# ibrahimhroob/SPS

Hardware: AMD Instinct MI355X
Metric: scans/sec @100k pts, 0.1 m voxel (higher is better)
Workload: dtype f32; 1 GPU; BASELINE config 2: single ~100k-pt LiDAR-like scan + variant-B submap, 0.1 m voxel, CustomMinkUNet14 fp32, 1 scan per step per GPU (4 distinct scans cycled); scan_points=100824, rows=153557, streams_per_gpu=8, compact_arenas=True

## Files before the change

sps_amd/csrc/conv_kernels.inc.h:

```cpp

typedef float floatx4 __attribute__((ext_vector_type(4)));

struct ConvArgs {
  const float *in;
  float *out;
  const float *Wu;
  const float *scale;
  const float *shift;
  const float *res;
  const int *nbr;
  const uint32_t *tmask;
  const int *n_out;
  const int *abort_flag;
  int out_rows;
  int64_t ldn;
  int ldi, ldo, ldr;
  int K, cin, cout, NT, upk;
  int relu, S;
  float inv_upk;
  float in_const;
  uint32_t in_bytes, wu_bytes, nbr_bytes;
  int tile_cap;
  int trace_on;
  const float *in2;
// ... 706 lines not shown
        yv[i] = y;
        if (UP) acc_s[0][rr * AST + col] = y;
      }
      if (ro < count && c0 < a.cout) {
        float *__restrict__ op = a.out + (size_t)ro * a.ldo + c0;
        if constexpr (EP_CPT == 2) *reinterpret_cast<float2 *>(op) = make_float2(yv[0], yv[1]);
        else *reinterpret_cast<float4 *>(op) = make_float4(yv[0], yv[1], yv[2], yv[3]);
      }
      if (FIN) {
#pragma unroll
        for (int o = 1; o < EP_TPR; o <<= 1) fsum += __shfl_xor(fsum, o, 64);
        if ((threadIdx.x % EP_TPR) == 0 && ro < count) a.fin_out[ro] = fsum + a.fin_b;
      }
    }
    if constexpr (UP) {
      __syncthreads();
      const __amdgpu_buffer_rsrc_t rsU = __builtin_amdgcn_make_buffer_rsrc((void *)a.up_Wu, 0, (int)a.up_wu_bytes, 0x00020000);
      const float usc = n < a.up_cout ? a.up_scale[n] : 0.f, ush = n < a.up_cout ? a.up_shift[n] : 0.f;
      const __amdgpu_buffer_rsrc_t rsUm = __builtin_amdgcn_make_buffer_rsrc((void *)a.up_tmask, 0, (int)0xFFFFFFFEu, 0x00020000);
      uint32_t om[4];
      const uint32_t omv = __builtin_amdgcn_raw_buffer_load_b32(rsUm, row0 + 16 * q < count ? (uint32_t)(st * 4 + q) * 16u : 0xFFFFFFFFu, 0, 0) & 0xFFu;
#pragma unroll
      for (int t = 0; t < 4; ++t) om[t] = (uint32_t)__builtin_amdgcn_readlane((int)omv, 16 * t);
#pragma unroll
      for (int kk = 0; kk < 2; ++kk) {
        const int k = 2 * wave + kk;
        if (!(((om[0] | om[1] | om[2] | om[3]) >> k) & 1u)) continue;
        const u32x4 vb = __builtin_amdgcn_raw_buffer_load_b128(rsU, (uint32_t)(k * 4 + q) * 256u + (uint32_t)n * 16u, 0, 0);
#pragma unroll
        for (int t = 0; t < 4; ++t) {
          if (!((om[t] >> k) & 1u)) continue;
          int child[4];
          {
            const int4 cv4 = *reinterpret_cast<const int4 *>(a.up_down + (size_t)k * a.up_ldn + row0 + 16 * t + q * 4);
            const int cv[4] = {cv4.x, cv4.y, cv4.z, cv4.w};
#pragma unroll
            for (int i = 0; i < 4; ++i) {
              const int ro = row0 + 16 * t + q * 4 + i;
              child[i] = ro < count ? cv[i] : -1;
              if (child[i] >= a.up_rows) child[i] = -1;
            }
          }
          const floatx4 xa = *reinterpret_cast<const floatx4 *>(acc_s[0] + (16 * t + n) * AST + 4 * q);
          floatx4 d = floatx4{0.f, 0.f, 0.f, 0.f};
          d = __builtin_amdgcn_mfma_f32_16x16x4f32(xa.x, __uint_as_float(vb.x), d, 0, 0, 0);
          d = __builtin_amdgcn_mfma_f32_16x16x4f32(xa.y, __uint_as_float(vb.y), d, 0, 0, 0);
          d = __builtin_amdgcn_mfma_f32_16x16x4f32(xa.z, __uint_as_float(vb.z), d, 0, 0, 0);
          d = __builtin_amdgcn_mfma_f32_16x16x4f32(xa.w, __uint_as_float(vb.w), d, 0, 0, 0);
          if (n < a.up_cout) {
#pragma unroll
            for (int i = 0; i < 4; ++i)
              if (child[i] >= 0) a.up_out[(size_t)child[i] * a.up_ldo + n] = fmaxf(d[i] * usc + ush, 0.f);
          }
        }
      }
    }
    PX_STAMP(6);
#if defined(SPS_WAVE_TRACE)
    if (tr_on && lane == 0 && st < 4096) {
      tr[7] = ((unsigned long long)nch << 32) | (unsigned)st;
      if (wave < 4) for (int i = 0; i < 8; ++i) g_px_trace[(st * 4 + wave) * 8 + i] = tr[i];
    }
#endif
    __syncthreads();
  }
}

template <int NT>
__global__ __launch_bounds__(256) void k_upconv(ConvArgs a) {
  if (a.abort_flag && *a.abort_flag) return;
  const int count = *a.n_out;
  const int ntiles = (count + 15) >> 4;
  const int lane = threadIdx.x & 63, wave = __builtin_amdgcn_readfirstlane((int)(threadIdx.x >> 6));
  const int r = lane & 15, q = lane >> 4;
  const __amdgpu_buffer_rsrc_t rsA = __builtin_amdgcn_make_buffer_rsrc((void *)a.in, 0, (int)a.in_bytes, 0x00020000);
  const __amdgpu_buffer_rsrc_t rsW = __builtin_amdgcn_make_buffer_rsrc((void *)a.Wu, 0, (int)a.wu_bytes, 0x00020000);
  const int upk = a.upk;
  const int ngrp = (upk + 3) >> 2;
  float esc[NT], esh[NT];
#pragma unroll
  for (int nt = 0; nt < NT; ++nt) {
    const int col = nt * 16 + r;
    esc[nt] = col < a.cout ? a.scale[col] : 0.f;
    esh[nt] = col < a.cout ? a.shift[col] : 0.f;
  }
  for (int tile = blockIdx.x; tile < ntiles; tile += gridDim.x) {
    const int row0 = tile * 16;
    const uint32_t mask = a.tmask[(size_t)tile * 4] & 0xFFu;
    const int row = row0 + r;
    u32x4 va[4];
#pragma unroll
    for (int i = 0; i < 4; ++i) {
      const uint32_t oa = (i < ngrp && 4 * i + q < upk && row < count) ? (uint32_t)row * ((uint32_t)a.ldi * 4u) + (uint32_t)(4 * i + q) * 16u : OOR;
      va[i] = __builtin_amdgcn_raw_buffer_load_b128(rsA, oa, 0, 0);
    }
#pragma unroll
    for (int kk = 0; kk < 2; ++kk) {
      const int k = 2 * wave + kk;
      if (!((mask >> k) & 1u)) continue;
      int child[4];
      {
        const int4 cv4 = *reinterpret_cast<const int4 *>(a.nbr + (size_t)k * a.ldn + row0 + q * 4);
        const int cv[4] = {cv4.x, cv4.y, cv4.z, cv4.w};
#pragma unroll
        for (int i = 0; i < 4; ++i) {
          const int ro = row0 + q * 4 + i;
          child[i] = ro < count ? cv[i] : -1;
          if (a.out_rows > 0 && child[i] >= a.out_rows) child[i] = -1;
        }
      }
      floatx4 acc[NT];
#pragma unroll
      for (int nt = 0; nt < NT; ++nt) acc[nt] = floatx4{0.f, 0.f, 0.f, 0.f};
#pragma unroll
      for (int i = 0; i < 4; ++i) {
        if (i >= ngrp) break;
        const uint32_t ob = 4 * i + q < upk ? ((uint32_t)(k * upk + 4 * i + q) * (uint32_t)NT) * 256u + (uint32_t)r * 16u : OOR;
        u32x4 vb[NT];
#pragma unroll
        for (int nt = 0; nt < NT; ++nt) vb[nt] = __builtin_amdgcn_raw_buffer_load_b128(rsW, ob + nt * 256u, 0, 0);
#pragma unroll
        for (int nt = 0; nt < NT; ++nt) {
          acc[nt] = __builtin_amdgcn_mfma_f32_16x16x4f32(__uint_as_float(va[i].x), __uint_as_float(vb[nt].x), acc[nt], 0, 0, 0);
          acc[nt] = __builtin_amdgcn_mfma_f32_16x16x4f32(__uint_as_float(va[i].y), __uint_as_float(vb[nt].y), acc[nt], 0, 0, 0);
          acc[nt] = __builtin_amdgcn_mfma_f32_16x16x4f32(__uint_as_float(va[i].z), __uint_as_float(vb[nt].z), acc[nt], 0, 0, 0);
          acc[nt] = __builtin_amdgcn_mfma_f32_16x16x4f32(__uint_as_float(va[i].w), __uint_as_float(vb[nt].w), acc[nt], 0, 0, 0);
        }
      }
      const __amdgpu_buffer_rsrc_t rsR = __builtin_amdgcn_make_buffer_rsrc((void *)(a.res ? a.res : a.out), 0, (int)0xFFFFFFFEu, 0x00020000);
#pragma unroll
      for (int nt = 0; nt < NT; ++nt) {
        const int col = nt * 16 + r;
        if (col >= a.cout) continue;
        float rv[4] = {0.f, 0.f, 0.f, 0.f};
        if (a.res) {
#pragma unroll
          for (int i = 0; i < 4; ++i)
            rv[i] = __uint_as_float(__builtin_amdgcn_raw_buffer_load_b32(
                rsR, child[i] >= 0 ? ((uint32_t)child[i] * (uint32_t)a.ldr + (uint32_t)col) * 4u : 0xFFFFFFFFu, 0, 0));
        }
#pragma unroll
        for (int i = 0; i < 4; ++i) {
          if (child[i] < 0) continue;
          float y = acc[nt][i] * esc[nt] + esh[nt];
          y += rv[i];
          if (a.relu) y = fmaxf(y, 0.f);
          a.out[(size_t)child[i] * a.ldo + col] = y;
        }
      }
    }
  }
}

__global__ __launch_bounds__(256) void k_conv0_fused(const int *__restrict__ n_out, LevelView L,
                                                      const float *__restrict__ W, const float *__restrict__ scale,
                                                      const float *__restrict__ shift, float in_const,
                                                      float *__restrict__ out, int ldo, int relu, TileOrderArgs to, int g0) {
  __shared__ float w_s[128 * 8];
  const int gto = (int)gridDim.x - g0;
  if ((int)blockIdx.x < gto) {
    const int which = (int)blockIdx.x;
    if (which < NLV - TILE_ORDER_FIRST_LEVEL)
      tile_order_body(to, which);
    else
      px_order_body(to, which - (NLV - TILE_ORDER_FIRST_LEVEL));
    return;
  }
  const int bid = (int)blockIdx.x - gto;
  if (n_out[ABORT]) return;
  for (int i = threadIdx.x; i < 128 * 8; i += blockDim.x) w_s[i] = i < 125 * 8 ? W[i] : 0.f;
  __syncthreads();
  const int n = *n_out;
  const int ntiles = (n + 15) >> 4;
  const int lane = threadIdx.x & 63, wave = __builtin_amdgcn_readfirstlane((int)(threadIdx.x >> 6));
  const int r = lane & 15, q = lane >> 4;
  const float esc = r < 8 ? scale[r] : 0.f, esh = r < 8 ? shift[r] : 0.f;
  const __amdgpu_buffer_rsrc_t rsM = __builtin_amdgcn_make_buffer_rsrc((void *)L.bmask, 0, (int)0xFFFFFFFEu, 0x00020000);
  for (int tile = bid * 4 + wave; tile < ntiles; tile += g0 * 4) {
    const int row0 = tile * 16;
    const int u = row0 + r;
    uint32_t bm[4] = {0u, 0u, 0u, 0u};
#if defined(SPS_ABLATE_C0FETCH)
    bm[0] = bm[1] = 0x0F0F0F0Fu;
    if (false) {
      const int blk = L.vblock[u];
#else
    if (u < n) {
      const int blk = L.vblock[u];
#endif
      const int bit = L.vbit[u];
      const int px = bit & 3, py = (bit >> 2) & 3, pz = bit >> 4;
      const int lx = px < 2 ? -1 : 0, ly = py < 2 ? -1 : 0, lz = pz < 2 ? -1 : 0;
      const int ysel = q & 1, zsel = q >> 1;
      const int *adj = L.badj + (size_t)blk * 81 + 27 + (lz + zsel + 1) * 9 + (ly + ysel + 1) * 3 + (lx + 1);
      const int nb0 = adj[0], nb1 = adj[1];
      const u32x2 M0 = __builtin_amdgcn_raw_buffer_load_b64(rsM, nb0 >= 0 ? (uint32_t)nb0 * 8u : 0xFFFFFFFFu, 0, 0);
      const u32x2 M1 = __builtin_amdgcn_raw_buffer_load_b64(rsM, nb1 >= 0 ? (uint32_t)nb1 * 8u : 0xFFFFFFFFu, 0, 0);
      const uint32_t m0lo = M0.x, m0hi = M0.y, m1lo = M1.x, m1hi = M1.y;
      const int ysplit = 4 * (ly + 1), zsplit = 4 * (lz + 1);
      const int ty0 = ysel ? ysplit : py - 2, ty1 = ysel ? py + 2 : ysplit - 1;
      const int tz0 = zsel ? zsplit : pz - 2, tz1 = zsel ? pz + 2 : zsplit - 1;
      const int xs = px - 2 - 4 * lx;
#pragma unroll 1
      for (int iz = 0; iz < 4; ++iz) {
        const int tz = tz0 + iz;
        const bool hiw = (tz & 2) != 0;
        const uint32_t w0 = hiw ? m0hi : m0lo, w1 = hiw ? m1hi : m1lo;
        uint32_t plane = 0u;
#pragma unroll
        for (int iy = 0; iy < 4; ++iy) {
          const int ty = ty0 + iy;
          const bool on = tz <= tz1 && ty <= ty1;
          const int sh = ((tz & 1) << 4) | ((ty & 3) << 2);
          const uint32_t n0 = (w0 >> sh) & 0xFu, n1 = (w1 >> sh) & 0xFu;
          const uint32_t pres = on ? (((n0 | (n1 << 4)) >> xs) & 0x1Fu) : 0u;
          plane |= pres << (5 * iy);
        }
        const int k0 = 5 * ((ty0 - py + 2) + 5 * (tz - pz + 2));
        const unsigned long long wide = (unsigned long long)plane << (k0 & 31);
        const int wi = (k0 >> 5) & 3;
        bm[0] |= wi == 0 ? (uint32_t)wide : 0u;
        bm[1] |= wi == 1 ? (uint32_t)wide : (wi == 0 ? (uint32_t)(wide >> 32) : 0u);
        bm[2] |= wi == 2 ? (uint32_t)wide : (wi == 1 ? (uint32_t)(wide >> 32) : 0u);
        bm[3] |= wi == 3 ? (uint32_t)wide : (wi == 2 ? (uint32_t)(wide >> 32) : 0u);
      }
    }
#pragma unroll
    for (int w = 0; w < 4; ++w) {
      bm[w] |= __shfl_xor(bm[w], 16, 64);
      bm[w] |= __shfl_xor(bm[w], 32, 64);
    }
    floatx4 acc = floatx4{0.f, 0.f, 0.f, 0.f};
    uint32_t bq[4];
#pragma unroll
    for (int w = 0; w < 4; ++w) bq[w] = bm[w] >> q;
    const uint32_t cbits = __float_as_uint(in_const);
#pragma unroll
    for (int g = 0; g < 32; ++g) {
      const int k = 4 * g + q;
      const float av = __uint_as_float((uint32_t)__builtin_amdgcn_sbfe((int)bq[g >> 3], (4 * g) & 31, 1) & cbits);
      const float bv = r < 8 ? w_s[k * 8 + r] : 0.f;
      acc = __builtin_amdgcn_mfma_f32_16x16x4f32(av, bv, acc, 0, 0, 0);
    }
    if (r < 8) {
#pragma unroll
      for (int i = 0; i < 4; ++i) {
        const int ro = row0 + q * 4 + i;
        if (ro < n) {
          const float y = acc[i] * esc + esh;
          out[(size_t)ro * ldo + r] = relu ? fmaxf(y, 0.f) : y;
        }
      }
    }
  }
}


constexpr double FEAT_FIX = 4294967296.0;

__global__ void k_voxel_feat_accum(const float *__restrict__ feats, const int *__restrict__ inv, int n,
                                   long long *__restrict__ vacc, int *__restrict__ vcnt, const int *__restrict__ n_dev) {
  if (n_dev) n = min(n, *n_dev);
  const int p = blockIdx.x * blockDim.x + threadIdx.x;
  if (p >= n) return;
  const int v = inv[p];
  if (v < 0) return;
  const double f = fmin(fmax((double)feats[p], -32768.0), 32768.0);
  atomicAdd(reinterpret_cast<unsigned long long *>(vacc) + v, (unsigned long long)__double2ll_rn(f * FEAT_FIX));
  atomicAdd(vcnt + v, 1);
}

__global__ void k_voxel_feat_mean(const int *__restrict__ n_vox, const long long *__restrict__ vacc,
                                  const int *__restrict__ vcnt, float *__restrict__ vfeat) {
  if (n_vox[ABORT]) return;
  const int n = *n_vox;
  for (int v = blockIdx.x * blockDim.x + threadIdx.x; v < n; v += gridDim.x * blockDim.x)
    vfeat[v] = (float)(((double)vacc[v] / FEAT_FIX) / (double)max(vcnt[v], 1));
}

__global__ __launch_bounds__(256) void k_conv0_feat(const int *__restrict__ n_out, LevelView L,
                                                     const float *__restrict__ W, const float *__restrict__ scale,
                                                     const float *__restrict__ shift,
                                                     const float *__restrict__ vfeat, float *__restrict__ out,
                                                     int ldo, TileOrderArgs to, int g0) {
  __shared__ float w_s[128 * 8];
  __shared__ float val_s[4][16][132];
  const int gto = (int)gridDim.x - g0;
  if ((int)blockIdx.x < gto) {
    const int which = (int)blockIdx.x;
    if (which < NLV - TILE_ORDER_FIRST_LEVEL)
      tile_order_body(to, which);
    else
      px_order_body(to, which - (NLV - TILE_ORDER_FIRST_LEVEL));
    return;
  }
  const int bid = (int)blockIdx.x - gto;
  if (n_out[ABORT]) return;
  for (int i = threadIdx.x; i < 128 * 8; i += blockDim.x) w_s[i] = i < 125 * 8 ? W[i] : 0.f;
  __syncthreads();
  const int n = *n_out;
  const int ntiles = (n + 15) >> 4;
  const int lane = threadIdx.x & 63, wave = __builtin_amdgcn_readfirstlane((int)(threadIdx.x >> 6));
  const int r = lane & 15, q = lane >> 4;
  const float esc = r < 8 ? scale[r] : 0.f, esh = r < 8 ? shift[r] : 0.f;
  float *va = val_s[wave][r];
  for (int tile = bid * 4 + wave; tile < ntiles; tile += g0 * 4) {
    const int row0 = tile * 16;
    const int u = row0 + r;
    __builtin_amdgcn_wave_barrier();
    for (int j = q; j < 128; j += 4) va[j] = 0.f;
    __builtin_amdgcn_wave_barrier();
    if (u < n) {
      const int blk = L.vblock[u];
      const int bit = L.vbit[u];
      const int px = bit & 3, py = (bit >> 2) & 3, pz = bit >> 4;
      const int *adj = L.badj + (size_t)blk * 81;
      for (int c = q; c < 25; c += 4) {
        const int ty = py + c % 5 - 2, tz = pz + c / 5 - 2;
        const int ad0 = 27 + ((tz >> 2) + 1) * 9 + ((ty >> 2) + 1) * 3 + 1;
        const int nbit0 = ((tz & 3) << 4) | ((ty & 3) << 2);
        int last_bo = 99, base = 0;
        unsigned long long mk = 0ull;
#pragma unroll
        for (int dx = -2; dx <= 2; ++dx) {
          const int tx = px + dx;
          const int bo = tx >> 2;
          if (bo != last_bo) {
            last_bo = bo;
            const int nb = adj[ad0 + bo];
            mk = nb >= 0 ? L.bmask[nb] : 0ull;
            base = nb >= 0 ? L.bbase[nb] : 0;
          }
          const int nbit = nbit0 | (tx & 3);
          if ((mk >> nbit) & 1ull) va[5 * c + dx + 2] = vfeat[base + __popcll(mk & ((1ull << nbit) - 1ull))];
        }
      }
    }
    __builtin_amdgcn_wave_barrier();
    floatx4 acc = floatx4{0.f, 0.f, 0.f, 0.f};
#pragma unroll
    for (int g = 0; g < 32; ++g) {
      const int k = 4 * g + q;
      const float av = va[k];
      const float bv = r < 8 ? w_s[k * 8 + r] : 0.f;
      acc = __builtin_amdgcn_mfma_f32_16x16x4f32(av, bv, acc, 0, 0, 0);
    }
    if (r < 8) {
#pragma unroll
      for (int i = 0; i < 4; ++i) {
        const int ro = row0 + q * 4 + i;
        if (ro < n) out[(size_t)ro * ldo + r] = fmaxf(acc[i] * esc + esh, 0.f);
      }
    }
  }
}

__global__ void k_slice_head(const float *__restrict__ F, int ldf, const int *__restrict__ inv, int n,
                             const float *__restrict__ W, const float *__restrict__ bias, int oc, int act,
                             float *__restrict__ out, int64_t ldo, const int *__restrict__ abort_flag,
                             const int *__restrict__ n_dev) {
  if (n_dev) n = min(n, *n_dev);
  const int p = blockIdx.x * blockDim.x + threadIdx.x;
  if (p >= n) return;
  const int v = (abort_flag && *abort_flag) ? -1 : inv[p];
  float f[8];
  if (v >= 0) {
    const float4 a = *reinterpret_cast<const float4 *>(F + (size_t)v * ldf);
    const float4 b = *reinterpret_cast<const float4 *>(F + (size_t)v * ldf + 4);
    f[0] = a.x, f[1] = a.y, f[2] = a.z, f[3] = a.w, f[4] = b.x, f[5] = b.y, f[6] = b.z, f[7] = b.w;
  }
  for (int j = 0; j < oc; ++j) {
    float y = __builtin_nanf("");
    if (v >= 0) {
      y = 0.f;
#pragma unroll
      for (int c = 0; c < 8; ++c) y += f[c] * W[c * oc + j];
      y += bias[j];
      if (act == 1) y = 1.0f / (1.0f + expf(-y));
    }
    out[(size_t)p * ldo + j] = y;
  }
}

__global__ void k_slice_sigmoid(const float *__restrict__ logits, const int *__restrict__ inv, int n,
                                float *__restrict__ scores, const int *__restrict__ abort_flag) {
  const int p = blockIdx.x * blockDim.x + threadIdx.x;
  if (p >= n) return;
  const int v = (abort_flag && *abort_flag) ? -1 : inv[p];
  scores[p] = v >= 0 ? 1.0f / (1.0f + expf(-logits[v])) : __builtin_nanf("");
}

__global__ __launch_bounds__(256) void k_bhash_cleanup(PyramidArgs pa, int gb) {
  bhash_cleanup(pa, (int)blockIdx.x / gb, (int)blockIdx.x % gb, gb);
}
```

sps_amd/csrc/sps_hip.hip:

```cpp
#include <hip/hip_runtime.h>

#include <cmath>
#include <cstdarg>
#include <cstdint>
#include <cstdio>
#include <algorithm>
#include <array>
#include <cstdlib>
#include <cstring>
#include <map>
#include <memory>
#include <string>
#include <vector>

#include "../../include/sps_hip.h"

#if !defined(SPS_DIAG)
#undef SPS_ABLATE_A
#undef SPS_ABLATE_B
#undef SPS_ABLATE_HALF_B
#undef SPS_ABLATE_SKIP_B
#undef SPS_ABLATE_MFMA
#undef SPS_ABLATE_LOOP
#undef SPS_ABLATE_STAGE
// ... 430 lines not shown

PyramidArgs pyramid_args(sps_ctx *c) {
  PyramidArgs a{};
  for (int l = 0; l < NLV; ++l) {
    const Level &L = c->lv[l];
    a.h[l] = L.h;
    a.sslot[l] = L.sslot;
    a.bslot[l] = L.bslot;
    a.bkey[l] = L.bkey;
    a.bmask[l] = L.bmask;
    a.bbase[l] = L.bbase;
    a.bmb[l] = L.bmb;
    a.bparent[l] = L.bparent;
    a.bchild[l] = L.bchild;
    a.badj[l] = L.badj;
    a.vblock[l] = L.vblock;
    a.vbit[l] = L.vbit;
  }
  a.counts = c->counts;
  a.sbit0 = c->lv[0].sbit;
  a.agg = c->scan_agg;
  a.agg_stride = (int)(c->cap / SCAN_BLOCK + 8);
  a.gen = (uint32_t)(c->fwd_gen % 0xFFFFFFFFull) + 1u;
  a.n_dev = nullptr;
  for (int l = 0; l < NLV; ++l) {
    a.capl[l] = (int)c->capl[l];
    a.bcapl[l] = (int)c->bcapl[l];
  }
  a.err = c->err;
  return a;
}

struct Map {
  const int *nbr;
  const uint32_t *tmask;
};

struct ConvCall {
  const char *name;
  const float *in;
  int ldi;
  float *out;
  int ldo;
  Map map;
  int level_out;
  const float *res;
  int ldr;
  int relu;
  const float *in2 = nullptr;
  int ldi2 = 0;
  bool fin = false;
  const char *up = nullptr;
  float *up_out = nullptr;
  int up_ldo = 0;
};

#ifndef SPS_FUSE_UP
#define SPS_FUSE_UP 12
#endif
constexpr int FUSE_UP = SPS_FUSE_UP;

struct Geometry {
  int ntw, S;
};
Geometry conv_geometry(int level, int K, int cin, int nt, int64_t cap = 0, bool serial_chain = false) {
  if (K == 8 && level >= 3) return {std::min(2, nt), 4};
  if (K == 1 || K == 8) return {nt <= 2 ? nt : 1, 1};
  (void)cin;
  Geometry g = level <= 1 ? Geometry{nt, 1} : Geometry{std::min(2, nt), 4};
  if (serial_chain && K == 81 && level >= 3 && nt >= 2 && cap > 0) {
    const int64_t tiles = std::max<int64_t>(1, cap * (level == 3 ? 33 : 11) / 1000 / 16);
    if (tiles * nt <= 800) g.ntw = 1;
  }
#if defined(SPS_DIAG)
  struct Hook {
    bool set = false;
    int ntw = 1, S = 1;
  };
  static const std::array<Hook, SPS_NUM_LEVELS> hooks = [] {
    std::array<Hook, SPS_NUM_LEVELS> h{};
    for (int l = 0; l < SPS_NUM_LEVELS; ++l) {
      char name[32];
      snprintf(name, sizeof name, "SPS_GEOM_L%d", l);
      const char *e = diag_env(name);
      int ntw = 1, S = 1;
      if (e && sscanf(e, "%d,%d", &ntw, &S) == 2 && (S == 1 || S == 2 || S == 4 || S == 8) && (ntw == 1 || ntw == 2 || ntw == 4))
        h[l] = Hook{true, ntw, S};
    }
    return h;
  }();
  if (level >= 0 && level < SPS_NUM_LEVELS && hooks[level].set) g = {std::min(hooks[level].ntw, nt), hooks[level].S};
#endif
  return g;
}

template <int NW, int CIN, bool C8, bool DS, bool FIN, int MINW, bool UP = false, bool HALF = false>
void launch_px(dim3 grid, hipStream_t st, const ConvArgs &a) {
  hipLaunchKernelGGL((k_conv_px<NW, CIN, C8, DS, FIN, MINW, UP, HALF>), grid, dim3(NW * 64), 0, st, a);
}

int launch_k_conv(const ConvArgs &a, Geometry g, bool ds, dim3 grid, hipStream_t st, unsigned lds_pad = 0) {
  if (a.up_out) {
    const int cgs = a.NT / g.ntw;
    const int unt = (a.up_cout + 15) / 16;
    if (!(g.ntw == 2 && g.S == 4 && ds)) return fail(SPS_ERR_INVALID, "fused transposed convolution: geometry ntw = %d, S = %d", g.ntw, g.S);
    if (cgs == 1 && unt == 1)
      hipLaunchKernelGGL((k_conv<2, SPS_G2, 4, true, false, 4, 1, 1, true>), grid, dim3(256), lds_pad, st, a);
    else if (cgs == 2 && unt == 2)
      hipLaunchKernelGGL((k_conv<2, SPS_G2, 4, true, false, 4, 2, 2, true>), grid, dim3(512), lds_pad, st, a);
    else if (cgs == 2 && unt == 4)
      hipLaunchKernelGGL((k_conv<2, SPS_G2, 4, true, false, 4, 2, 4, true>), grid, dim3(512), lds_pad, st, a);
    else
      return fail(SPS_ERR_INVALID, "fused transposed convolution: no instantiation for %d column groups, %d output tiles", cgs, unt);
    return SPS_OK;
  }
#define SPS_LAUNCH(NTW_, G_, W_, S_)                                                              \
  do {                                                                                            \
    if (ds)                                                                                       \
      hipLaunchKernelGGL((k_conv<NTW_, G_, W_, true, false, S_>), grid, dim3(S_ == 8 ? 512 : 256), lds_pad, st, a);     \
    else                                                                                          \
      hipLaunchKernelGGL((k_conv<NTW_, G_, W_, false, false, S_>), grid, dim3(S_ == 8 ? 512 : 256), lds_pad, st, a);    \
  } while (0)
#define SPS_LAUNCH_U4(NTW_, G_, W_)                                                                               \
  do {                                                                                                            \
    if (ds)                                                                                                       \
      hipLaunchKernelGGL((k_conv<NTW_, G_, W_, true, false, 4, 1, 0, true>), grid, dim3(256), lds_pad, st, a);    \
    else                                                                                                          \
      hipLaunchKernelGGL((k_conv<NTW_, G_, W_, false, false, 4, 1, 0, true>), grid, dim3(256), lds_pad, st, a);   \
  } while (0)
  if (g.S == 4 && (a.upk & 3) == 0 && a.upk > 0 && (!ds || (a.upk2 & 3) == 0)) {
    if (g.ntw == 1) { SPS_LAUNCH_U4(1, SPS_G1, SPS_WS); return SPS_OK; }
    if (g.ntw == 2) { SPS_LAUNCH_U4(2, SPS_G2, SPS_W2); return SPS_OK; }
  }
#undef SPS_LAUNCH_U4
  const int key = g.ntw * 10 + g.S;
  switch (key) {
    case 11: SPS_LAUNCH(1, SPS_G1, SPS_W1, 1); break;
    case 12: SPS_LAUNCH(1, SPS_G1, SPS_WS, 2); break;
    case 14: SPS_LAUNCH(1, SPS_G1, SPS_WS, 4); break;
    case 21: SPS_LAUNCH(2, SPS_G2, SPS_W2, 1); break;
    case 22: SPS_LAUNCH(2, SPS_G2, SPS_W2, 2); break;
    case 24: SPS_LAUNCH(2, SPS_G2, SPS_W2, 4); break;
    case 18: SPS_LAUNCH(1, SPS_G1, 3, 8); break;
    case 28: SPS_LAUNCH(2, SPS_G2, 3, 8); break;
    case 41: SPS_LAUNCH(4, SPS_G4, SPS_W4, 1); break;
    case 42: SPS_LAUNCH(4, SPS_G4, SPS_W4, 2); break;
    case 44: SPS_LAUNCH(4, SPS_G4, SPS_W4, 4); break;
    default: return fail(SPS_ERR_INVALID, "unsupported conv geometry ntw = %d, S = %d", g.ntw, g.S);
  }
#undef SPS_LAUNCH
  return SPS_OK;
}

int run_conv(sps_ctx *c, const ConvCall &cc, hipStream_t st) {
  const NetSpec &s = *c->net;
  const int ci = s.find_conv(cc.name);
  if (ci < 0) return fail(SPS_ERR_INVALID, "unknown conv %s", cc.name);
  const ConvSpec &cs = s.convs[ci];
  ConvArgs a{};
  a.in = cc.in;
  a.ldi = cc.ldi;
  a.out = cc.out;
  a.ldo = cc.ldo;
  a.Wu = c->wu + cs.wu_off;
  a.scale = c->ss + cs.ss_off;
  a.shift = c->ss + cs.ss_off + cs.cout;
  a.res = cc.res;
  a.ldr = cc.ldr;
  a.nbr = cc.map.nbr;
  a.tmask = cc.map.tmask;
  a.ldn = c->capl[cc.level_out];
  a.n_out = c->counts + cc.level_out;
  a.abort_flag = c->counts + 15;
  a.K = cs.K;
  a.cin = cs.cin;
  a.cout = cs.cout;
  a.NT = cs.nt();
  a.upk = cs.upk();
  a.inv_upk = cs.cin >= 4 ? 1.0f / (float)cs.upk() : 1.f;
  a.relu = cc.relu;
  a.in_const = 0.5f;
  const Geometry g = conv_geometry(cc.level_out, cs.K, cs.cin, a.NT, (int64_t)c->cap, !c->pipelined);
  a.S = g.S;
  int64_t gx = (c->cap / 64) >> cc.level_out;
  if (gx < 64) gx = 64;
  if (gx > 4096) gx = 4096;
  {
    static const float gscale = [] { const char *e = diag_env("SPS_GRID_SCALE"); return e ? (float)atof(e) : 1.f; }();
    if (gscale != 1.f) gx = std::max<int64_t>(16, (int64_t)((float)gx * gscale));
  }
  static const int max_wg = [] { const char *e = diag_env("SPS_CONV_MAX_WG"); return e ? atoi(e) : 0; }();
  if (max_wg > 0 && gx * (a.NT / g.ntw) * g.S > max_wg) gx = std::max<int64_t>(16, max_wg / ((a.NT / g.ntw) * g.S));
  dim3 grid((unsigned)(a.NT / g.ntw), (unsigned)(gx * g.S), 1u);
  a.in2 = cc.in2;
  a.ldi2 = cc.ldi2;
  a.upk2 = cs.ds_cin / 4;
  a.in2_bytes = (uint32_t)((size_t)c->capl[cc.level_out] * (size_t)(cc.ldi2 > 0 ? cc.ldi2 : 1) * 4u);
  if (cs.ds_cin > 0 && !cc.in2) return fail(SPS_ERR_INVALID, "%s needs the block input for its fused downsample", cc.name);
  if (cc.fin) {
    const ConvSpec &fs = s.convs[s.find_conv("final")];
    a.fin_w = c->blob + fs.w_off;
    a.fin_b = c->final_bias;
    a.fin_out = c->logits;
  }
  const bool is_up = cs.K == 8 && std::strncmp(cc.name, "convtr", 6) == 0;
  const int level_in = cs.K == 8 ? (is_up ? cc.level_out + 1 : cc.level_out - 1) : cc.level_out;
  a.in_bytes = (uint32_t)((size_t)c->capl[level_in < 0 ? 0 : level_in] * (size_t)cc.ldi * 4u);
  a.wu_bytes = (uint32_t)(cs.wu_numel() * 4);
  a.nbr_bytes = (uint32_t)((size_t)cs.K * (size_t)c->capl[cc.level_out] * 4u);
  a.tile_cap = (int)(c->capl[cc.level_out] / 16);
  a.tile_order = (TILE_ORDER != 0 && cs.K == 81 && cc.level_out >= TILE_ORDER_FIRST_LEVEL) ? c->lv[cc.level_out].tile_order : nullptr;
  a.order_ways = TILE_ORDER == 2 ? TILE_ORDER_WAYS / std::max(1, a.NT / g.ntw) : 0;
  if (cc.up) {
    const ConvSpec &us = s.convs[s.find_conv(cc.up)];
    if (us.cin != cs.cout || cc.level_out < 1) return fail(SPS_ERR_INVALID, "%s cannot be fused into %s", cc.up, cc.name);
    a.up_Wu = c->wu + us.wu_off;
    a.up_scale = c->ss + us.ss_off;
    a.up_shift = c->ss + us.ss_off + us.cout;
    a.up_down = c->lv[cc.level_out].down;
    a.up_tmask = c->lv[cc.level_out].tmdown;
    a.up_ldn = c->capl[cc.level_out];
    a.up_out = cc.up_out;
    a.up_ldo = cc.up_ldo;
    a.up_cout = us.cout;
    a.up_rows = (int)c->capl[cc.level_out - 1];
    a.up_wu_bytes = (uint32_t)(us.wu_numel() * 4);
    grid.x = 1;
    a.order_ways = TILE_ORDER == 2 ? TILE_ORDER_WAYS : 0;
  }
  {
    static const char *trace_layer = diag_env("SPS_TRACE_LAYER");
    a.trace_on = trace_layer && std::strcmp(trace_layer, cc.name) == 0;
  }
  if (cs.cin == 1) {
    TileOrderArgs to{};
    const int g0 = grid_for(c->cap, 64, 4096);
    int gto = 0;
    if (TILE_ORDER != 0) {
      for (int l = 0; l < NLV; ++l) {
        const bool px = l < PX_LEVELS && ((px_levels() >> l) & 1) && c->lv[l].px_order;
        to.tm3[l] = (c->lv[l].nbr3 || !px) ? c->lv[l].tm3 : nullptr, to.order[l] = c->lv[l].tile_order;
        to.rb_cnt[l] = px ? c->lv[l].rb_cnt : nullptr, to.px_sorted[l] = c->lv[l].px_sorted, to.px_order[l] = c->lv[l].px_order;
      }
      to.counts = c->counts;
      gto = NLV - TILE_ORDER_FIRST_LEVEL + PX_LEVELS;
    }
    c->last_kernel = c->cur_vfeat ? "k_conv0_feat" : "k_conv0_fused";
    {
      static const int c0mode = [] { const char *e = diag_env("SPS_DIAG_CONV0"); return e ? atoi(e) : 0; }();
      if (c0mode == 1) {
        hipLaunchKernelGGL(k_conv0_fused, dim3((unsigned)gto), dim3(256), 0, st, a.n_out, c->lv[0].view(), c->blob + cs.w_off, a.scale,
                           a.shift, a.in_const, a.out, a.ldo, 1, to, 0);
        return SPS_OK;
      }
      if (c0mode == 2) gto = 0;
    }
    if (c->cur_vfeat) {
      hipLaunchKernelGGL(k_conv0_feat, dim3((unsigned)(g0 + gto)), dim3(256), 0, st, a.n_out,
                         c->lv[0].view(), c->blob + cs.w_off, a.scale, a.shift, c->cur_vfeat, a.out, a.ldo, to, g0);
      return SPS_OK;
    }
    hipLaunchKernelGGL(k_conv0_fused, dim3((unsigned)(g0 + gto)), dim3(256), 0, st, a.n_out,
                       c->lv[0].view(), c->blob + cs.w_off, a.scale, a.shift, a.in_const, a.out, a.ldo, 1, to, g0);
    return SPS_OK;
  }
  if (cs.K == 8 && std::strncmp(cc.name, "convtr", 6) == 0) {
    {
      const int coarse = cc.level_out + 1;
      a.nbr = c->lv[coarse].down;
      a.tmask = c->lv[coarse].tmdown;
      a.n_out = c->counts + coarse;
      a.ldn = c->capl[coarse];
      a.tile_cap = (int)(c->capl[coarse] / 16);
      a.out_rows = (int)c->capl[cc.level_out];
      int64_t gu = (c->cap / 16) >> coarse;
      if (gu < 64) gu = 64;
      if (gu > 8192) gu = 8192;
      const dim3 gr((unsigned)gu);
      c->last_kernel = "k_upconv";
      if (a.NT == 1)
        hipLaunchKernelGGL((k_upconv<1>), gr, dim3(256), 0, st, a);
      else if (a.NT == 2)
        hipLaunchKernelGGL((k_upconv<2>), gr, dim3(256), 0, st, a);
      else
        hipLaunchKernelGGL((k_upconv<4>), gr, dim3(256), 0, st, a);
      return SPS_OK;
    }
  }
  const bool ds = cs.ds_cin > 0;
  if (cc.level_out < PX_LEVELS && ((px_levels() >> cc.level_out) & 1) && c->lv[cc.level_out].rb_e && cs.K == 81 && a.NT == 1 && (cs.cout == 8 || cs.cout == 16) &&
      (cs.cin == 8 || cs.cin == 16 || cs.cin == 24) && (!cc.fin || cs.cout == 8)) {
    int64_t gs = (c->cap / 64) >> cc.level_out;
    if (gs < 64) gs = 64;
    if (gs > 4096) gs = 4096;
    const dim3 gridp((unsigned)gs);
    a.rb_e = c->lv[cc.level_out].rb_e;
    a.rb_k = c->lv[cc.level_out].rb_k;
    a.rb_cnt = c->lv[cc.level_out].rb_cnt;
    a.px_order = TILE_ORDER != 0 ? c->lv[cc.level_out].px_order : nullptr;
    a.rb_supertiles = (int)(c->capl[cc.level_out] / 64);
    const int key = cs.cin * 100 + (cs.cout == 8 ? 10 : 0) + (cc.fin ? 2 : (ds ? 1 : 0));
    c->last_kernel = "k_conv_px";
    static_assert(PX_HALF_LEVELS == 1, "SPS_PX_LAUNCH picks the HALF instantiations for level 0 alone");
    if (px_half_level(cc.level_out) && cs.cout != 8)
      return fail(SPS_ERR_INVALID, "%s: C_out = %d cannot read the 8-pair rulebook of level %d", cc.name, cs.cout, cc.level_out);
#define SPS_PX_LAUNCH(CIN_, C8_, DS_, FIN_)                                                                  \
  do {                                                                                                       \
    if (cc.level_out == 0)                                                                                   \
      launch_px<SPS_PX0, CIN_, C8_, DS_, FIN_, SPS_PX0_W, false, C8_>(gridp, st, a);                         \
    else                                                                                                     \
      launch_px<SPS_PX1, CIN_, C8_, DS_, FIN_, SPS_PX1_W>(gridp, st, a);                                     \
  } while (0)
    switch (key) {
      case 800: SPS_PX_LAUNCH(8, false, false, false); break;
      case 810: SPS_PX_LAUNCH(8, true, false, false); break;
      case 811: SPS_PX_LAUNCH(8, true, true, false); break;
      case 812: SPS_PX_LAUNCH(8, true, true, true); break;
      case 1601:
        if (cc.up) {
          if (cc.level_out != 1 || a.up_cout > 16) return fail(SPS_ERR_INVALID, "%s cannot be fused into %s", cc.up, cc.name);
          launch_px<SPS_PX1, 16, false, true, false, SPS_PX1_W, true>(gridp, st, a);
        } else {
          SPS_PX_LAUNCH(16, false, true, false);
        }
        break;
      case 1610: SPS_PX_LAUNCH(16, true, false, false); break;
      case 2400: SPS_PX_LAUNCH(24, false, false, false); break;
      default: return fail(SPS_ERR_INVALID, "no k_conv_px instantiation for %s", cc.name);
    }
#undef SPS_PX_LAUNCH
    return SPS_OK;
  }
  if (cs.K == 81 && !a.nbr)
    return fail(SPS_ERR_INVALID, "%s has no pair-exact instantiation and the inference-only context keeps no neighbour table at level %d",
                cc.name, cc.level_out);
  if (cc.fin && !(g.ntw == 1 && ds && g.S == 1)) return fail(SPS_ERR_INVALID, "final fusion needs NT = 1, S = 1");
  c->last_kernel = cs.K == 81 ? (cc.level_out >= 2 ? "k_conv<3x3x3x3, levels 2-4>" : "k_conv<3x3x3x3, levels 0-1>") : "k_conv<2x2x2x1 stride 2>";
  if (cc.fin) {
    hipLaunchKernelGGL((k_conv<1, SPS_G1DS, SPS_W1, true, true, 1>), grid, dim3(256), 0, st, a);
    return SPS_OK;
  }
  unsigned lds_pad = 0;
#if defined(SPS_DIAG)
  {
    static const int pad = [] { const char *e = diag_env("SPS_CONV_LDS_PAD"); return e ? atoi(e) : 0; }();
    if (cc.level_out >= 2 && cs.K == 81) lds_pad = (unsigned)pad;
  }
#endif
  return launch_k_conv(a, g, ds, grid, st, lds_pad);
}

void permute_weights(const ConvSpec &cs, const float *W, float *Wu, const float *colscale = nullptr) {
  if (cs.cin == 1) {
    for (int k = 0; k < cs.K; ++k)
      for (int n = 0; n < 16; ++n) Wu[k * 16 + n] = n < cs.cout ? W[(size_t)k * cs.cout + n] : 0.f;
    return;
  }
  const int upk = cs.upk(), NT = cs.nt();
  for (int k = 0; k < cs.K; ++k)
    for (int c4 = 0; c4 < upk; ++c4) {
      const int u = k * upk + c4;
      for (int nt = 0; nt < NT; ++nt)
        for (int n = 0; n < 16; ++n)
          for (int sidx = 0; sidx < 4; ++sidx) {
            const int col = nt * 16 + n;
            float v = col < cs.cout ? W[((size_t)k * cs.cin + 4 * c4 + sidx) * cs.cout + col] : 0.f;
            if (colscale && col < cs.cout) v *= colscale[col];
            Wu[(((size_t)u * NT + nt) * 16 + n) * 4 + sidx] = v;
          }
    }
}

void prof_mark(sps_ctx *c, const char *name, hipStream_t st) {
  if (!c->prof) return;
  if (c->prof_n >= c->prof_ev.size()) {
    hipEvent_t e;
    if (hipEventCreate(&e) != hipSuccess) return;
    c->prof_ev.push_back(e);
    c->prof_names.emplace_back();
    c->prof_kernels.emplace_back();
  }
  c->prof_names[c->prof_n] = name;
  c->prof_kernels[c->prof_n] = c->last_kernel;
  c->last_kernel = "";
  (void)hipEventRecord(c->prof_ev[c->prof_n], st);
  ++c->prof_n;
}

std::vector<Feat> feature_taps(sps_ctx *c) {
  return {
      {"out_p1", c->cat8 + 8, 16, 8, 0},  {"block1", c->cat7 + 16, 24, 8, 1}, {"block2", c->cat6 + 32, 48, 16, 2},
      {"block3", c->cat5 + 64, 96, 32, 3}, {"block4", c->b4o, 64, 64, 4},      {"block5", c->b5o, 64, 64, 3},
      {"block6", c->b6o, 32, 32, 2},       {"block7", c->b7o, 16, 16, 1},      {"block8", c->b8o, 8, 8, 0},
  };
}

template <typename TIN>
int radius_item_launch(sps_ctx *c, const TIN *scan, int64_t ld, int64_t n, const int32_t *row_off_dev, ItemOut io,
                              int32_t *n_rows_dev, hipStream_t st) {
  const int64_t n27 = n * 27;
  const int nb = (int)((n27 + PSCAN_BLOCK - 1) / PSCAN_BLOCK);
  const unsigned gq = (unsigned)((n27 + 255) / 256);
  hipLaunchKernelGGL((k_item_scan_rows<TIN>), dim3((unsigned)((n + 255) / 256)), dim3(256), 0, st, scan, ld, (int)n, row_off_dev, io);
  hipLaunchKernelGGL((k_radius_query<TIN, 0>), dim3(gq), dim3(256), 0, st, scan, ld, (int)n, c->rg, c->item_counts, nullptr,
                     nullptr, nullptr, ItemOut{});
  hipLaunchKernelGGL(k_scan_partial, dim3((unsigned)nb), dim3(256), 0, st, c->item_counts, n27, c->item_bsum);
  hipLaunchKernelGGL(k_scan_top, dim3(1), dim3(256), 0, st, c->item_bsum, nb, row_off_dev, (int)n, io.row_cap, c->item_base,
                     n_rows_dev, c->err);
  hipLaunchKernelGGL(k_scan_apply, dim3((unsigned)nb), dim3(256), 0, st, c->item_counts, n27, c->item_bsum, c->item_offsets);
  io.row_base = c->item_base;
  hipLaunchKernelGGL((k_radius_query<TIN, 2>), dim3(gq), dim3(256), 0, st, scan, ld, (int)n, c->rg, nullptr, nullptr, nullptr,
                     c->item_offsets, io);
  return SPS_OK;
}

struct RowWrite {
  float t = 1.f;
  float *feat = nullptr;
  float feat_value = 0.f;
  const int *n_dev = nullptr;
};

template <typename TIN>
int transform_launch(const TIN *in, int64_t ld, int64_t n, const Mat4 &T, int identity, void *out, int out_f64,
                            bool with_bt, int64_t ldo, const RowWrite &rw, hipStream_t st) {
  const dim3 g((unsigned)((n + 255) / 256)), b(256);
  if (with_bt)
    hipLaunchKernelGGL((k_transform_points<TIN, float, true>), g, b, 0, st, in, ld, (int)n, T, identity, (float *)out, ldo,
                       rw.t, rw.feat, rw.feat_value, rw.n_dev);
  else if (out_f64)
    hipLaunchKernelGGL((k_transform_points<TIN, double, false>), g, b, 0, st, in, ld, (int)n, T, identity, (double *)out, ldo,
                       rw.t, nullptr, 0.f, rw.n_dev);
  else
    hipLaunchKernelGGL((k_transform_points<TIN, float, false>), g, b, 0, st, in, ld, (int)n, T, identity, (float *)out, ldo,
                       rw.t, nullptr, 0.f, rw.n_dev);
  return SPS_OK;
}

}

// ... 1195 lines not shown
```

Measured before the change: 4098 scans/s.

## Add dedicated k_down kernel for stride-2 K=8 downsampling convolutions

Adds a specialized MFMA kernel for stride-2 (K=8) convolutions that builds a compact list of active kernel offsets per tile from the tile mask and splits the reduction across waves with an LDS reduction when S=4. It replaces the generic conv path for these layers by default. An optional compile flag can instead host the tile-order bodies in the conv1p1s2 launch rather than the conv0 launch. The new path rejects unsupported geometries with an error, which risks failures for configurations it does not cover.

```diff
diff --git a/sps_amd/csrc/conv_kernels.inc.h b/sps_amd/csrc/conv_kernels.inc.h
--- a/sps_amd/csrc/conv_kernels.inc.h
+++ b/sps_amd/csrc/conv_kernels.inc.h
@@ -882,11 +882,154 @@
   }
 }
 
+#ifndef SPS_ORDER_HOST
+#define SPS_ORDER_HOST 0
+#endif
+#ifndef SPS_DOWN_KERNEL
+#define SPS_DOWN_KERNEL 1
+#endif
+static_assert(SPS_ORDER_HOST == 0 || SPS_DOWN_KERNEL == 1, "the conv1p1s2 launch hosts the order bodies only as k_down");
+
+template <int UPK, int NT, int S, bool HOST>
+__global__ __launch_bounds__(256) void k_down(ConvArgs a, TileOrderArgs to, int gto) {
+  static_assert(S == 1 || S == 4, "a wave per tile or a workgroup per tile");
+  static_assert((UPK & (UPK - 1)) == 0, "C_in / 4 a power of two");
+  constexpr int MAXG = ((8 * UPK + S - 1) / S + 3) / 4;
+  static_assert(MAXG <= 4, "register budget: four operand sets");
+  constexpr int LOGU = UPK == 1 ? 0 : UPK == 2 ? 1 : UPK == 4 ? 2 : UPK == 8 ? 3 : 4;
+  if constexpr (HOST) {
+    if ((int)blockIdx.x < gto) {
+      const int which = (int)blockIdx.x;
+      if (which < NLV - TILE_ORDER_FIRST_LEVEL)
+        tile_order_body(to, which);
+      else
+        px_order_body(to, which - (NLV - TILE_ORDER_FIRST_LEVEL));
+      return;
+    }
+  }
+  const int bid = (int)blockIdx.x - (HOST ? gto : 0), nblk = (int)gridDim.x - (HOST ? gto : 0);
+  constexpr int tpw = 4 / S;
+  const int lane = threadIdx.x & 63, wave = __builtin_amdgcn_readfirstlane((int)(threadIdx.x >> 6));
+  const int r = lane & 15, q = lane >> 4;
+  const int tl = S == 1 ? wave : 0, split = S == 1 ? 0 : wave;
+  const __amdgpu_buffer_rsrc_t rsA = __builtin_amdgcn_make_buffer_rsrc((void *)a.in, 0, (int)a.in_bytes, 0x00020000);
+  const __amdgpu_buffer_rsrc_t rsW = __builtin_amdgcn_make_buffer_rsrc((void *)a.Wu, 0, (int)a.wu_bytes, 0x00020000);
+  const __amdgpu_buffer_rsrc_t rsN = __builtin_amdgcn_make_buffer_rsrc((void *)a.nbr, 0, (int)a.nbr_bytes, 0x00020000);
+  const uint32_t ldn32 = (uint32_t)a.ldn;
+  const uint32_t ldi4 = (uint32_t)a.ldi * 4u;
+  constexpr uint32_t wunit = (uint32_t)NT * 256u;
+  const int cnt = *a.n_out;
+  const int aborted = *a.abort_flag;
+  uint32_t m = 0u;
+  int d[8];
+  const __amdgpu_buffer_rsrc_t rsM = __builtin_amdgcn_make_buffer_rsrc((void *)a.tmask, 0, a.tile_cap * 16, 0x00020000);
+  auto fetch = [&](int tile) {
+    m = __builtin_amdgcn_raw_buffer_load_b32(rsM, (uint32_t)tile * 16u, 0, 0);
+#pragma unroll
+    for (int k = 0; k < 8; ++k)
+      d[k] = (int)__builtin_amdgcn_raw_buffer_load_b32(rsN, ((uint32_t)k * ldn32 + (uint32_t)(tile * 16 + r)) * 4u, 0, 0);
+  };
+  fetch(bid * tpw + tl);
+  float esc[NT], esh[NT];
+#pragma unroll
+  for (int nt = 0; nt < NT; ++nt) {
+    const int col = nt * 16 + r;
+    esc[nt] = col < a.cout ? a.scale[col] : 0.f;
+    esh[nt] = col < a.cout ? a.shift[col] : 0.f;
+  }
+  const int count = aborted ? 0 : cnt;
+  const int ntiles = min((count + 15) >> 4, a.tile_cap);
+  __shared__ float red_s[S > 1 ? (S - 1) * NT * 4 * 64 : 1];
+  for (int grp = bid; grp * tpw < ntiles; grp += nblk) {
+    const int tile = grp * tpw + tl;
+    if (S == 1 && tile >= ntiles) continue;
+    if (grp != bid) fetch(tile);
+    const int row0 = tile * 16;
+    const uint32_t mk = (uint32_t)__builtin_amdgcn_readfirstlane((int)m) & 0xFFu;
+    uint32_t kl = 0u;
+    int nk = 0;
+#pragma unroll
+    for (int k = 0; k < 8; ++k)
+      if ((mk >> k) & 1u) kl |= (uint32_t)k << (4 * nk), ++nk;
+    const int U = nk * UPK;
+    int per = (U + S - 1) / S;
+    per = (per + 3) & ~3;
+    const int j0 = split * per;
+    const int j1 = min(U, j0 + per);
+    const bool rv = row0 + r < count;
+    u32x4 va[MAXG];
+    u32x4 vb[MAXG][NT];
+#pragma unroll
+    for (int g = 0; g < MAXG; ++g) {
+      const int j = j0 + 4 * g + q;
+      const bool valid = j < j1;
+      const int p = min(j >> LOGU, 7), c4 = j & (UPK - 1);
+      const int k = (int)((kl >> (4 * p)) & 7u);
+      int child = d[0];
+#pragma unroll
+      for (int kk = 1; kk < 8; ++kk) child = k == kk ? d[kk] : child;
+      const uint32_t oa = (valid && rv && child >= 0) ? (uint32_t)child * ldi4 + (uint32_t)c4 * 16u : OOR;
+      const uint32_t ob = valid ? (uint32_t)(k * UPK + c4) * wunit + (uint32_t)r * 16u : OOR;
+      va[g] = __builtin_amdgcn_raw_buffer_load_b128(rsA, oa, 0, 0);
+#pragma unroll
+      for (int nt = 0; nt < NT; ++nt) vb[g][nt] = __builtin_amdgcn_raw_buffer_load_b128(rsW, ob + nt * 256u, 0, 0);
+    }
+    floatx4 acc[NT];
+#pragma unroll
+    for (int nt = 0; nt < NT; ++nt) acc[nt] = floatx4{0.f, 0.f, 0.f, 0.f};
+#pragma unroll
+    for (int g = 0; g < MAXG; ++g) {
+      if (j0 + 4 * g >= j1) break;
+#pragma unroll
+      for (int nt = 0; nt < NT; ++nt) {
+        acc[nt] = __builtin_amdgcn_mfma_f32_16x16x4f32(__uint_as_float(va[g].x), __uint_as_float(vb[g][nt].x), acc[nt], 0, 0, 0);
+        acc[nt] = __builtin_amdgcn_mfma_f32_16x16x4f32(__uint_as_float(va[g].y), __uint_as_float(vb[g][nt].y), acc[nt], 0, 0, 0);
+        acc[nt] = __builtin_amdgcn_mfma_f32_16x16x4f32(__uint_as_float(va[g].z), __uint_as_float(vb[g][nt].z), acc[nt], 0, 0, 0);
+        acc[nt] = __builtin_amdgcn_mfma_f32_16x16x4f32(__uint_as_float(va[g].w), __uint_as_float(vb[g][nt].w), acc[nt], 0, 0, 0);
+      }
+    }
+    if constexpr (S > 1) {
+      if (grp != bid) __syncthreads();
+      if (split != 0) {
+        float *rd = red_s + (split - 1) * (NT * 4 * 64) + lane;
+#pragma unroll
+        for (int nt = 0; nt < NT; ++nt)
+#pragma unroll
+          for (int i = 0; i < 4; ++i) rd[(nt * 4 + i) * 64] = acc[nt][i];
+      }
+      __syncthreads();
+      if (split != 0) continue;
+      for (int sp = 1; sp < S; ++sp) {
+        const float *rd = red_s + (sp - 1) * (NT * 4 * 64) + lane;
+#pragma unroll
+        for (int nt = 0; nt < NT; ++nt)
+#pragma unroll
+          for (int i = 0; i < 4; ++i) acc[nt][i] += rd[(nt * 4 + i) * 64];
+      }
+    }
+#pragma unroll
+    for (int nt = 0; nt < NT; ++nt) {
+      const int col = nt * 16 + r;
+      if (col >= a.cout) continue;
+      const float sc = esc[nt], sh = esh[nt];
+#pragma unroll
+      for (int i = 0; i < 4; ++i) {
+        const int ro = row0 + q * 4 + i;
+        if (ro >= count) continue;
+        float y = acc[nt][i] * sc + sh;
+        if (a.relu) y = fmaxf(y, 0.f);
+        a.out[(size_t)ro * a.ldo + col] = y;
+      }
+    }
+  }
+}
+
 __global__ __launch_bounds__(256) void k_conv0_fused(const int *__restrict__ n_out, LevelView L,
                                                       const float *__restrict__ W, const float *__restrict__ scale,
                                                       const float *__restrict__ shift, float in_const,
                                                       float *__restrict__ out, int ldo, int relu, TileOrderArgs to, int g0) {
   __shared__ float w_s[128 * 8];
+#if SPS_ORDER_HOST == 0
   const int gto = (int)gridDim.x - g0;
   if ((int)blockIdx.x < gto) {
     const int which = (int)blockIdx.x;
@@ -897,6 +1040,10 @@
     return;
   }
   const int bid = (int)blockIdx.x - gto;
+#else
+  (void)to;
+  const int bid = (int)blockIdx.x;
+#endif
   if (n_out[ABORT]) return;
   for (int i = threadIdx.x; i < 128 * 8; i += blockDim.x) w_s[i] = i < 125 * 8 ? W[i] : 0.f;
   __syncthreads();
@@ -1015,6 +1162,7 @@
                                                      int ldo, TileOrderArgs to, int g0) {
   __shared__ float w_s[128 * 8];
   __shared__ float val_s[4][16][132];
+#if SPS_ORDER_HOST == 0
   const int gto = (int)gridDim.x - g0;
   if ((int)blockIdx.x < gto) {
     const int which = (int)blockIdx.x;
@@ -1025,6 +1173,10 @@
     return;
   }
   const int bid = (int)blockIdx.x - gto;
+#else
+  (void)to;
+  const int bid = (int)blockIdx.x;
+#endif
   if (n_out[ABORT]) return;
   for (int i = threadIdx.x; i < 128 * 8; i += blockDim.x) w_s[i] = i < 125 * 8 ? W[i] : 0.f;
   __syncthreads();
diff --git a/sps_amd/csrc/sps_hip.hip b/sps_amd/csrc/sps_hip.hip
--- a/sps_amd/csrc/sps_hip.hip
+++ b/sps_amd/csrc/sps_hip.hip
@@ -606,6 +606,17 @@
   return SPS_OK;
 }
 
+int order_args(sps_ctx *c, TileOrderArgs &to) {
+  if (TILE_ORDER == 0) return 0;
+  for (int l = 0; l < NLV; ++l) {
+    const bool px = l < PX_LEVELS && ((px_levels() >> l) & 1) && c->lv[l].px_order;
+    to.tm3[l] = (c->lv[l].nbr3 || !px) ? c->lv[l].tm3 : nullptr, to.order[l] = c->lv[l].tile_order;
+    to.rb_cnt[l] = px ? c->lv[l].rb_cnt : nullptr, to.px_sorted[l] = c->lv[l].px_sorted, to.px_order[l] = c->lv[l].px_order;
+  }
+  to.counts = c->counts;
+  return NLV - TILE_ORDER_FIRST_LEVEL + PX_LEVELS;
+}
+
 int run_conv(sps_ctx *c, const ConvCall &cc, hipStream_t st) {
   const NetSpec &s = *c->net;
   const int ci = s.find_conv(cc.name);
@@ -689,18 +700,9 @@
   if (cs.cin == 1) {
     TileOrderArgs to{};
     const int g0 = grid_for(c->cap, 64, 4096);
-    int gto = 0;
-    if (TILE_ORDER != 0) {
-      for (int l = 0; l < NLV; ++l) {
-        const bool px = l < PX_LEVELS && ((px_levels() >> l) & 1) && c->lv[l].px_order;
-        to.tm3[l] = (c->lv[l].nbr3 || !px) ? c->lv[l].tm3 : nullptr, to.order[l] = c->lv[l].tile_order;
-        to.rb_cnt[l] = px ? c->lv[l].rb_cnt : nullptr, to.px_sorted[l] = c->lv[l].px_sorted, to.px_order[l] = c->lv[l].px_order;
-      }
-      to.counts = c->counts;
-      gto = NLV - TILE_ORDER_FIRST_LEVEL + PX_LEVELS;
-    }
+    int gto = SPS_ORDER_HOST == 0 ? order_args(c, to) : 0;
     c->last_kernel = c->cur_vfeat ? "k_conv0_feat" : "k_conv0_fused";
-    {
+    if (SPS_ORDER_HOST == 0) {
       static const int c0mode = [] { const char *e = diag_env("SPS_DIAG_CONV0"); return e ? atoi(e) : 0; }();
       if (c0mode == 1) {
         hipLaunchKernelGGL(k_conv0_fused, dim3((unsigned)gto), dim3(256), 0, st, a.n_out, c->lv[0].view(), c->blob + cs.w_off, a.scale,
@@ -740,6 +742,25 @@
         hipLaunchKernelGGL((k_upconv<4>), gr, dim3(256), 0, st, a);
       return SPS_OK;
     }
+  }
+  if (SPS_DOWN_KERNEL && cs.K == 8) {
+    if (cc.res || cs.ds_cin > 0 || cc.fin || cc.up || !a.nbr || !a.tmask) return fail(SPS_ERR_INVALID, "%s: k_down runs a plain stride-2 convolution", cc.name);
+    TileOrderArgs to{};
+    const int gto = (SPS_ORDER_HOST == 1 && std::strcmp(cc.name, "conv1p1s2") == 0) ? order_args(c, to) : 0;
+    const dim3 gd((unsigned)(gx * g.S + gto));
+    c->last_kernel = "k_down";
+    const int key = a.upk * 100 + a.NT * 10 + g.S;
+    if (key == 211 && gto > 0)
+      hipLaunchKernelGGL((k_down<2, 1, 1, true>), gd, dim3(256), 0, st, a, to, gto);
+    else if (key == 211)
+      hipLaunchKernelGGL((k_down<2, 1, 1, false>), gd, dim3(256), 0, st, a, to, 0);
+    else if (key == 414 && gto == 0)
+      hipLaunchKernelGGL((k_down<4, 1, 4, false>), gd, dim3(256), 0, st, a, to, 0);
+    else if (key == 824 && gto == 0)
+      hipLaunchKernelGGL((k_down<8, 2, 4, false>), gd, dim3(256), 0, st, a, to, 0);
+    else
+      return fail(SPS_ERR_INVALID, "no k_down instantiation for %s (C_in = %d, C_out = %d, %d splits)", cc.name, cs.cin, cs.cout, g.S);
+    return SPS_OK;
   }
   const bool ds = cs.ds_cin > 0;
   if (cc.level_out < PX_LEVELS && ((px_levels() >> cc.level_out) & 1) && c->lv[cc.level_out].rb_e && cs.K == 81 && a.NT == 1 && (cs.cout == 8 || cs.cout == 16) &&
```

Result: no change. 4096 scans/s (-0.0%).
